# RuntimeRacer/vall-e

Measured on AMD Instinct MI355X. Metric: AR codec-tokens/sec/GPU + NAR 7-stage p50 latency, d=1024 L=12 10s utterance, higher is better.
Workload: dtype bf16

## Files before the change

### include/vallex.h

```cpp
#ifndef VALLEX_H
#define VALLEX_H

#include <stdint.h>

#ifdef __cplusplus
extern "C" {
#endif

typedef struct vx_engine vx_engine;

enum vx_status {
  VX_OK = 0,
  VX_ERR_ARG = 1,
  VX_ERR_HIP = 2,
  VX_ERR_STATE = 3,
  VX_ERR_CAPACITY = 4,
  VX_ERR_UNSUPPORTED = 5,
  VX_ERR_WEIGHTS = 6
};

enum vx_precision {
  VX_PREC_F32 = 0,
  VX_PREC_BF16 = 1,
  VX_PREC_FP8_NAR = 2
// ... 105 lines not shown

int vx_get_timings(vx_engine* e, double* out, int32_t n);

int vx_read_buffer(vx_engine* e, const char* name, void* dst, int64_t offset_bytes, int64_t nbytes);

int vx_buffer_bytes(const vx_config* cfg, const char* name, int64_t* bytes);

int vx_op_layernorm(int32_t prec, const float* x, const float* gamma, const float* beta, const float* ada_w,
                    const float* ada_b, void* out , int32_t rows, int32_t d, void* stream);
int vx_op_gemv(int32_t prec, const void* W, const float* bias, const float* x, float* y, int32_t N, int32_t K,
               int32_t relu, void* stream);
int vx_op_gemm(int32_t prec, int32_t use_mfma, const void* A, const void* W, const float* bias, float* C_f32,
               int32_t M, int32_t N, int32_t K, int32_t relu, void* stream);
int vx_op_gemm_rows(int32_t form, const void* A_bf16, const void* W_bf16, const float* bias, void* C, int32_t M, int32_t N,
                    int32_t K, int32_t relu, void* vt_bf16, int32_t vt_n0, int32_t vt_ld, void* stream);
int vx_op_gemm_mx(const float* A, const float* W, const float* bias, void* c_out, void* sc_out, int32_t M, int32_t N, int32_t K,
                  int32_t relu, int32_t out_mode, void* qa_out, void* sa_out, void* stream);
int vx_op_layernorm_mx(const float* x, const float* gamma, const float* beta, const float* ada_w, const float* ada_b, void* q_out,
                       void* s_out, int32_t rows, int32_t d, void* stream);
int vx_op_attention(int32_t prec, int32_t use_mfma, const void* qkv, void* out, int32_t rows, int32_t nhead,
                    int32_t hd, int32_t text_len_for_ar_mask , void* stream);
int vx_op_attention_segs(const void* qkv, void* out, int32_t rows, int32_t nhead, int32_t hd, int32_t nseg, const int32_t* seg_start,
                         const int32_t* seg_len, const int32_t* seg_text , void* stream);
int vx_op_cross_attention_segs(const void* q, int32_t ldq, const void* mem, const int64_t* mem_off, int64_t head_stride,
                               int64_t v_offset, const int32_t* klen, void* out, int32_t rows, int32_t nhead, int32_t nseg,
                               const int32_t* seg_start, const int32_t* seg_len, void* stream);
int vx_op_attn_slots(int32_t kv_fp8, const float* q, const void* kv, const void* kv_scale, int64_t slot_stride, int64_t v_offset,
                     int32_t ctx_max, int32_t B, int32_t nhead, const int32_t* ctx, const int32_t* done , void* out,
                     void* stream);
int vx_op_attn_mem_slots(const float* q, const void* mem, int64_t slot_stride, int64_t v_offset, int32_t max_text, int32_t B,
// ... 75 lines not shown
```

### vall-e_amd/csrc/engine.hip

```cpp
#include <hip/hip_runtime.h>

#include <cmath>
#include <cstdarg>
#include <cstdio>
#include <array>
#include <cstring>
#include <string>
#include <type_traits>
#include <unordered_map>
#include <vector>

#include "../../include/vallex.h"
#ifdef VX_STAMPS
__device__ unsigned long long g_vx_stamps[32];
__device__ unsigned long long* g_vx_kstamps = nullptr;
__device__ unsigned long long* g_fq_stamps = nullptr;
#endif
#include "ar_kernels.hpp"
#include "ar_tp.hpp"
#include "rows_kernels.hpp"
#include "mfma_kernels.hpp"
#include "batch_kernels.hpp"
#include "mx_kernels.hpp"

// ... 2006 lines not shown
    for (int i = 0; i < Q - 1; ++i) {
      for (int b = 0; b < n; ++b) {
        float* xb = e->X + (size_t)start[b] * dn;
        float* xa = xb + (size_t)tx[b] * dn;
        const float* ye = e->yemb + (size_t)aoff[b] * dn;
        const int A = P[b] + T[b];
        if (prenet) {
          if (!vf) HIPC(hipMemcpyAsync(xb, e->pn_text, (size_t)S2[b] * dn * 4, hipMemcpyDeviceToDevice, e->es));
          if (pos_before_prenet) {
            add_pos_kernel<<<A, 256, 0, e->es>>>(ye, dn, a_aud, e->pe_nar, 0, e->pn_a, A);
            VXC(audio_prenet_rows(e, 1, e->pn_a, xa, A, dn));
          } else {
            VXC(audio_prenet_rows(e, 1, ye, e->pn_b, A, dn));
            add_pos_kernel<<<A, 256, 0, e->es>>>(e->pn_b, dn, a_aud, e->pe_nar, 0, xa, A);
          }
        } else {
          if (!vf) embed_pos_kernel<<<S2[b], 256, 0, e->es>>>(e->ids_text + soff[b], 1, 0, W<float>(e, "nar_text_embedding.word_embeddings.weight"),
                                                              512, dn, a_txt, e->pe_nar, 0, xb, S2[b]);
          add_pos_kernel<<<A, 256, 0, e->es>>>(ye, dn, a_aud, e->pe_nar, 0, xa, A);
        }
      }
      VXC(run_stack(e, e->nar_l, rows, dn, c.nar_nhead, -1, i, segs, KvDst(), tmem));
      const float* fw = post ? nullptr : ada_vec(e, i, e->npl * c.nar_num_layers);
      for (int b = 0; b < n; ++b) {
        const float* xr = e->X + (size_t)(start[b] + tx[b] + P[b]) * dn;
        void* hr = (char*)e->Hn + (size_t)toff[b] * dn * e->esz;
        if (post) VXC(cast_rows(e, xr, hr, (size_t)T[b] * dn));
        else VXC(ln_rows(e, xr, W<float>(e, "nar_decoder.norm.norm.weight"), W<float>(e, "nar_decoder.norm.norm.bias"), fw, fw + dn, hr,
                         T[b], dn));
      }
      VXC(gemm_rows(e, e->Hn, W<void>(e, "nar_predict_layers." + std::to_string(i) + ".weight"), nullptr, e->nar_logits,
                    trows, 1024, dn, GE_PLAIN, true));
      argmax_rows_kernel<<<(trows + 3) / 4, 256, 0, e->es>>>(e->nar_logits, 1024, trows, e->ids_samples, e->d_codes, Q, i + 1);
      if (score) {
        nll_rows_kernel<<<(trows + NLL_ROWS_PER_WG - 1) / NLL_ROWS_PER_WG, 256, 0, e->es>>>(e->nar_logits, trows, 1024, 1024, e->d_fcodes, Q, i + 1,
                                                                                   e->sc_nll, e->sc_rank, nullptr);
        for (int b = 0; b < n; ++b) {
          if (score->nll) HIPC(hipMemcpyAsync(score->nll[b] + (size_t)i * T[b], e->sc_nll + toff[b], (size_t)T[b] * 4, hipMemcpyDefault, e->es));
          if (score->rank) HIPC(hipMemcpyAsync(score->rank[b] + (size_t)i * T[b], e->sc_rank + toff[b], (size_t)T[b] * 4, hipMemcpyDefault, e->es));
        }
      }
      if (stage_logits) HIPC(hipMemcpyAsync(stage_logits + (size_t)i * trows * 1024, e->nar_logits, (size_t)trows * 1024 * 4, hipMemcpyDefault, e->es));
      if (forced && i < Q - 2)
        pick_col_kernel<<<(trows + 255) / 256, 256, 0, e->es>>>(e->d_fcodes, Q, i + 1, e->ids_samples, trows);
      if (i < Q - 2)
        for (int b = 0; b < n; ++b) {
          float* ye = e->yemb + (size_t)aoff[b] * dn;
          if (c.prefix_mode == 0 && P[b])
            embed_accum_kernel<<<P[b], 256, 0, e->es>>>(e->ids_prompts + (size_t)aoff[b] * Q, Q, i + 1, emb(i + 1), 1024, dn, ye, P[b], 0);
          embed_accum_kernel<<<T[b], 256, 0, e->es>>>(e->ids_samples + toff[b], 1, 0, emb(i + 1), 1024, dn, ye + (size_t)P[b] * dn, T[b], 0);
        }
    }
  }
  HIPC(hipGetLastError());
  HIPC(hipEventRecord(e->ev_t[5], e->es));
  for (int b = 0; codes_out && b < n; ++b)
    HIPC(hipMemcpyAsync(codes_out[b], e->d_codes + (size_t)toff[b] * Q, (size_t)T[b] * Q * 8, hipMemcpyDefault, e->es));
  HIPC(hipStreamSynchronize(e->es));
  float ms = 0.f;
  HIPC(hipEventElapsedTime(&ms, e->ev_t[4], e->ev_t[5]));
  e->t_nar = ms;
  gemm_collect(e);
  e->last_T = trows; e->last_N = rows;
  VXC(sync_out(e, stream));
  return VX_OK;
// ... 418 lines not shown

extern "C" int vx_op_gemm_rows(int32_t form, const void* A, const void* Wp, const float* bias, void* C, int32_t M, int32_t N,
                               int32_t K, int32_t relu, void* vt, int32_t vt_n0, int32_t vt_ld, void* stream) {
  if (!A || !Wp || !C || !bias || M < 1 || N < 1 || K < 1) return fail(VX_ERR_ARG, "gemm_rows: null operand or empty shape");
  if (form != 0 && form != 1) return fail(VX_ERR_ARG, "gemm_rows: form %d", form);
  if (vt && (form != 0 || vt_n0 < 0 || vt_n0 >= N || vt_n0 % 64 != 0 || vt_ld < M))
    return fail(VX_ERR_ARG, "gemm_rows: V^T copy needs form 0, 0 <= vt_n0 < N, vt_n0 %% 64 == 0 (the kernels test whole column groups), vt_ld >= M");
  hipStream_t s = (hipStream_t)stream;
  if (mfma_gemm_dispatch((const bf16*)A, (const bf16*)Wp, bias, C, M, N, K, form == 1 ? GE_RESID : (relu ? GE_RELU : GE_BIAS), form == 1, s,
                         (bf16*)vt, vt_n0, vt_ld))
    return fail(VX_ERR_UNSUPPORTED, "gemm_rows: no kernel instance");
  HIPC(hipGetLastError());
  return VX_OK;
}

extern "C" int vx_op_gemm_mx(const float* A, const float* Wt, const float* bias, void* c_out, void* sc_out, int32_t M, int32_t N,
                             int32_t K, int32_t relu, int32_t out_mode, void* qa_out, void* sa_out, void* stream) {
  if (!A || !Wt || !c_out || M < 1 || N % 256 || K % 128) return fail(VX_ERR_UNSUPPORTED, "mx gemm: M=%d N=%d K=%d (N %% 256, K %% 128)", M, N, K);
  if (out_mode == 2 && !sc_out) return fail(VX_ERR_ARG, "mx gemm: out_mode 2 needs sc_out");
  hipStream_t s = (hipStream_t)stream;
  const int ld = (M + 255) / 256 * 256;
  struct Scratch {
    uint8_t *qa = nullptr, *sa = nullptr, *qw = nullptr, *sw = nullptr;
    ~Scratch() { (void)hipFree(qa); (void)hipFree(sa); (void)hipFree(qw); (void)hipFree(sw); }
  } t;
  HIPC(hipMalloc((void**)&t.qa, (size_t)M * K)); HIPC(hipMalloc((void**)&t.sa, (size_t)(K / 32) * ld));
  HIPC(hipMalloc((void**)&t.qw, (size_t)N * K)); HIPC(hipMalloc((void**)&t.sw, (size_t)(K / 32) * N));
  HIPC(hipMemsetAsync(t.sa, 0, (size_t)(K / 32) * ld, s));
  mx_quant_rows_kernel<<<(M + 3) / 4, 256, 0, s>>>(A, t.qa, t.sa, M, K, ld);
  mx_quant_rows_kernel<<<(N + 3) / 4, 256, 0, s>>>(Wt, t.qw, t.sw, N, K, N);
// ... 406 lines not shown
```

### vall-e_amd/csrc/mfma_kernels.hpp

```cpp
#pragma once
#include <cstdlib>
#include <type_traits>
#include <unordered_map>

#include "common.hpp"
#include "rows_kernels.hpp"

namespace vx {

typedef __bf16 bf16x8_t __attribute__((ext_vector_type(8)));
typedef float f32x16_t __attribute__((ext_vector_type(16)));

template <int EPI, bool OUT_F32, int RING>
__global__ __launch_bounds__(256) void mfma_gemm_kernel(const bf16* __restrict__ A, const bf16* __restrict__ W,
                                                        const float* __restrict__ bias, void* __restrict__ Cv, int M,
                                                        int N, int K, bf16* __restrict__ vt, int vt_n0, int vt_ld, int ld) {
  const int bx = blockIdx.x, by = blockIdx.y, bz = blockIdx.z;
  A += (size_t)bz * K;
  W += (size_t)bz * K;
  if (OUT_F32) Cv = reinterpret_cast<float*>(Cv) + (size_t)bz * M * N;
  constexpr int BM = 128, BN = 128;
  extern __shared__ __attribute__((aligned(16))) unsigned char lds[];
  const int tid = threadIdx.x, lane = tid & 63, wave = tid >> 6;
  const int wm = wave >> 1, wn = wave & 1;
  const int r = lane & 31, h = lane >> 5;
  const int m0 = by * BM, n0 = bx * BN;

  f32x16_t acc[2][2];
// ... 15 lines not shown
  constexpr int KS = RK / 16;
  constexpr int OPB = BM * RB;
  constexpr int NI = OPB / 4096;
  constexpr int ND = 2 * NI;
  auto swz = [](int row) { return RB == 128 ? ((row >> 1) & 7) : ((0 - (row >> 2)) & 3); };
  const int nk = K / RK;
  const int row0 = tid / CPR;
  const int csrc = ((tid % CPR) ^ swz(row0)) * 8;
  const bf16 *sA[NI], *sW[NI];
#pragma unroll
  for (int i = 0; i < NI; ++i) {
    sA[i] = A + (size_t)min(m0 + row0 + (256 / CPR) * i, M - 1) * ld + csrc;
    sW[i] = W + (size_t)min(n0 + row0 + (256 / CPR) * i, N - 1) * ld + csrc;
  }
  const int dbase = (tid - lane) * 16;
  auto stage = [&](int st) {
    unsigned char* base = lds + (st & 3) * (2 * OPB);
    const int k0 = st * RK;
#pragma unroll
    for (int i = 0; i < NI; ++i)
      __builtin_amdgcn_global_load_lds((const __attribute__((address_space(1))) void*)(sA[i] + k0),
                                       (__attribute__((address_space(3))) void*)(base + dbase + 4096 * i), 16, 0, 0);
#pragma unroll
    for (int i = 0; i < NI; ++i)
      __builtin_amdgcn_global_load_lds((const __attribute__((address_space(1))) void*)(sW[i] + k0),
                                       (__attribute__((address_space(3))) void*)(base + OPB + dbase + 4096 * i), 16, 0, 0);
  };
  bf16x8_t fa0[KS][2], fb0[KS][2], fa1[KS][2], fb1[KS][2];
  auto lread = [&](int st, bf16x8_t (&fa)[KS][2], bf16x8_t (&fb)[KS][2]) {
    const unsigned char* ba = lds + (st & 3) * (2 * OPB);
    const unsigned char* bw = ba + OPB;
#pragma unroll
    for (int ks = 0; ks < KS; ++ks)
#pragma unroll
      for (int i = 0; i < 2; ++i) {
        const int row = wm * 64 + i * 32 + r;
        fa[ks][i] = *reinterpret_cast<const bf16x8_t*>(ba + row * RB + (((ks * 2 + h) ^ swz(row)) << 4));
        const int col = wn * 64 + i * 32 + r;
        fb[ks][i] = *reinterpret_cast<const bf16x8_t*>(bw + col * RB + (((ks * 2 + h) ^ swz(col)) << 4));
      }
  };
  auto mm = [&](const bf16x8_t (&fa)[KS][2], const bf16x8_t (&fb)[KS][2]) {
#pragma unroll
    for (int ks = 0; ks < KS; ++ks)
#pragma unroll
      for (int i = 0; i < 2; ++i)
#pragma unroll
        for (int j = 0; j < 2; ++j) acc[i][j] = __builtin_amdgcn_mfma_f32_32x32x16_bf16(fa[ks][i], fb[ks][j], acc[i][j], 0, 0, 0);
  };
  auto steady = [&](int st, bf16x8_t (&fa)[KS][2], bf16x8_t (&fb)[KS][2], bf16x8_t (&na)[KS][2], bf16x8_t (&nb)[KS][2]) {
    stage(st + 3);
    lread(st + 1, na, nb);
    mm(fa, fb);
#pragma unroll
    for (int i = 0; i < ND; ++i) {
      __builtin_amdgcn_sched_group_barrier(0x010, 1, 0);
      __builtin_amdgcn_sched_group_barrier(0x008, 1, 0);
    }
#pragma unroll
    for (int i = 0; i < 4 * KS - ND; ++i) {
      __builtin_amdgcn_sched_group_barrier(0x100, 4 * KS / (4 * KS - ND), 0);
      __builtin_amdgcn_sched_group_barrier(0x008, 1, 0);
    }
    if (ND == 8) asm volatile("s_waitcnt vmcnt(8)\n\ts_barrier" ::: "memory");
    else asm volatile("s_waitcnt vmcnt(4)\n\ts_barrier" ::: "memory");
  };
  auto tail = [&](int st, bf16x8_t (&fa)[KS][2], bf16x8_t (&fb)[KS][2], bf16x8_t (&na)[KS][2], bf16x8_t (&nb)[KS][2]) {
    const bool more = st + 3 < nk;
    if (more) stage(st + 3);
    if (st + 1 < nk) lread(st + 1, na, nb);
    mm(fa, fb);
    if (more && ND == 8) asm volatile("s_waitcnt vmcnt(8)\n\ts_barrier" ::: "memory");
    else if (more) asm volatile("s_waitcnt vmcnt(4)\n\ts_barrier" ::: "memory");
    else asm volatile("s_waitcnt vmcnt(0)\n\ts_barrier" ::: "memory");
  };
  VX_STAMP(0);
  const int pre = nk < 3 ? nk : 3;
  for (int st = 0; st < pre; ++st) stage(st);
  VX_STAMP(1);
  if (pre == 3 && ND == 8) asm volatile("s_waitcnt vmcnt(8)\n\ts_barrier" ::: "memory");
  else if (pre == 3) asm volatile("s_waitcnt vmcnt(4)\n\ts_barrier" ::: "memory");
  else asm volatile("s_waitcnt vmcnt(0)\n\ts_barrier" ::: "memory");
  lread(0, fa0, fb0);
  VX_STAMP(2);
  int st = 0;
  for (; st + 4 < nk; st += 2) {
    steady(st, fa0, fb0, fa1, fb1);
    steady(st + 1, fa1, fb1, fa0, fb0);
  }
  VX_STAMP(3);
  for (; st < nk; st += 2) {
    tail(st, fa0, fb0, fa1, fb1);
    if (st + 1 < nk) tail(st + 1, fa1, fb1, fa0, fb0);
  }
  VX_STAMP(4);
  asm volatile("" : "+v"(bias_r[0]), "+v"(bias_r[1]));

  if constexpr (!OUT_F32) {
    constexpr int LDT = 136;
    bf16* tile = reinterpret_cast<bf16*>(lds);
#pragma unroll
    for (int j = 0; j < 2; ++j) {
      const int nl = wn * 64 + j * 32 + r;
      const float bv = bias_r[j];
#pragma unroll
      for (int i = 0; i < 2; ++i)
#pragma unroll
        for (int v = 0; v < 16; ++v) {
          const int ml = wm * 64 + i * 32 + (v & 3) + 8 * (v >> 2) + 4 * h;
// ... 49 lines not shown
    for (int j = 0; j < 2; ++j) {
      const int n = n0 + wn * 64 + j * 32 + r;
      const float bv = bias_r[j];
#pragma unroll
      for (int i = 0; i < 2; ++i) {
#pragma unroll
        for (int v = 0; v < 16; ++v) {
          const int m = m0 + wm * 64 + i * 32 + (v & 3) + 8 * (v >> 2) + 4 * h;
          if (m < M && n < N) {
            float x = acc[i][j][v] + bv;
            if (EPI == GE_RELU) x = fmaxf(x, 0.f);
            float* c = reinterpret_cast<float*>(Cv) + (size_t)m * N + n;
            *c = (EPI == GE_RESID) ? (*c + x) : x;
          }
        }
      }
    }
  }
  VX_STAMP(5);
}

template <int EPI, bool OUT_F32, int SPLITK>
__global__ __launch_bounds__(256) void wgemm_kernel(const bf16* __restrict__ A, const bf16* __restrict__ W,
                                                    const float* __restrict__ bias, void* __restrict__ Cv, int M, int N,
                                                    int K, bf16* __restrict__ vt, int vt_n0, int vt_ld, int ngroups,
                                                    int ngroups_pad) {
  extern __shared__ __attribute__((aligned(16))) unsigned char lds[];
  const int tid = threadIdx.x, lane = tid & 63, wave = tid >> 6;
  const int r = lane & 31, h = lane >> 5;
  const int ng = blockIdx.x % ngroups_pad, mt = blockIdx.x / ngroups_pad;
// ... 625 lines not shown
  for (int c = 8; c >= 2; c >>= 1)
    if (rem * c <= grid && nk % (2 * c) == 0 && nk / c >= 8) { S = c; break; }
  if (S == 0) return tl;
  const float full = 1.5f * nk, split = 1.5f * nk / S + (float)rem * S * 0.262144f * 2.f / 4.f + 7.f;
  if (split > 0.7f * full) return tl;
  hipStreamCaptureStatus cs = hipStreamCaptureStatusNone;
  if (hipStreamIsCapturing(s, &cs) != hipSuccess || cs != hipStreamCaptureStatusNone) return tl;
  static std::unordered_map<hipStream_t, float*> wss;
  float*& w = wss[s];
  if (w == nullptr && hipMalloc((void**)&w, (size_t)256 * 262144) != hipSuccess) { w = nullptr; return tl; }
  tl.ws = w;
  tl.split = S;
  return tl;
}

static inline int mfma_gemm_dispatch(const bf16* A, const bf16* W, const float* bias, void* C, int M, int N, int K,
                                     int epi, bool out_f32, hipStream_t s, bf16* vt = nullptr, int vt_n0 = 0,
                                     int vt_ld = 0) {
  if (K % 64 != 0 || N % 64 != 0) {
    gemm_simple_launch(A, W, bias, C, M, N, K, epi, out_f32, s);
    return 0;
  }
  const long long tiles64 = (long long)((M + 63) / 64) * (N / 64);
  if (M >= 4096 && N % 256 == 0 && K >= 128) {
    const int ntn = N / 256, ntm = (M + 255) / 256, nt_all = ntn * ntm;
    const int ncu = vx_cu_count();
    const int grid256 = nt_all < ncu ? nt_all : ncu;
    const bool p8 = K % 128 == 0 && (size_t)M * K * 2 < 0xFFFF0000ull && (size_t)N * K * 2 < 0xFFFF0000ull;
    const P8Tail tl = p8 ? p8_tail_plan(nt_all, grid256, K, s) : P8Tail{nullptr, 0};
    gemm_epi_dispatch(epi, out_f32, [&](auto E, auto F) {
// ... 8 lines not shown
        attr_done = true;
      }
      if (p8 && tl.split > 1) {
        const int rem_t = nt_all % grid256;
        mfma256p_kernel<EPI, OUT_F32, true><<<grid256, 512, 131072 + 2048, s>>>(A, W, bias, C, M, N, K, vt, vt_n0, vt_ld, ntn, nt_all, tl);
        p8_tail_reduce_kernel<EPI, OUT_F32><<<dim3(rem_t, 16), 256, 0, s>>>(tl.ws, tl.split, nt_all - rem_t, ntn, nt_all, bias, C, M, N, vt, vt_n0, vt_ld);
      } else if (p8) {
        mfma256p_kernel<EPI, OUT_F32><<<grid256, 512, 131072 + 2048, s>>>(A, W, bias, C, M, N, K, vt, vt_n0, vt_ld, ntn, nt_all, tl);
      } else {
        mfma256_kernel<EPI, OUT_F32><<<grid256, 512, 131072, s>>>(A, W, bias, C, M, N, K, vt, vt_n0, vt_ld, ntn, nt_all);
      }
    });
    return 0;
  }
  if (N % 128 == 0 && tiles64 >= 512) {
    const dim3 grid(N / 128, (M + 127) / 128);
    const int ring = gemm_ring128((long long)grid.x * grid.y);
    gemm_epi_dispatch(epi, out_f32, [&](auto E, auto F) {
      constexpr int EPI = decltype(E)::value;
      constexpr bool OUT_F32 = decltype(F)::value;
      static bool attr_dev[16] = {};
      bool& attr_done = attr_dev[vx_cur_device()];
      if (!attr_done) {
        (void)hipFuncSetAttribute((const void*)mfma_gemm_kernel<EPI, OUT_F32, 64>, hipFuncAttributeMaxDynamicSharedMemorySize, 131072);
        (void)hipFuncSetAttribute((const void*)mfma_gemm_kernel<EPI, OUT_F32, 32>, hipFuncAttributeMaxDynamicSharedMemorySize, 65536);
        attr_done = true;
      }
      if (ring == 64) mfma_gemm_kernel<EPI, OUT_F32, 64><<<grid, 256, 131072, s>>>(A, W, bias, C, M, N, K, vt, vt_n0, vt_ld, K);
      else mfma_gemm_kernel<EPI, OUT_F32, 32><<<grid, 256, 65536, s>>>(A, W, bias, C, M, N, K, vt, vt_n0, vt_ld, K);
    });
    return 0;
  }
  const int mtiles = (M + 63) / 64;
  const size_t lds = 131072;
  const bool split = (K % 256 == 0) && tiles64 < 512;
  gemm_epi_dispatch(epi, out_f32, [&](auto E, auto F) {
    constexpr int EPI = decltype(E)::value;
    constexpr bool OUT_F32 = decltype(F)::value;
    auto launch = [&](auto SPLITK) {
      constexpr int S = decltype(SPLITK)::value;
      static bool attr_dev[16] = {};
      bool& attr_done = attr_dev[vx_cur_device()];
      if (!attr_done) {
        (void)hipFuncSetAttribute((const void*)wgemm_kernel<EPI, OUT_F32, S>, hipFuncAttributeMaxDynamicSharedMemorySize, (int)lds);
        attr_done = true;
      }
      const int ngr = (S == 1) ? (N + 255) / 256 : N / 64;
      const int ngp = (ngr + 7) / 8 * 8;
      wgemm_kernel<EPI, OUT_F32, S><<<mtiles * ngp, 256, lds, s>>>(A, W, bias, C, M, N, K, vt, vt_n0, vt_ld, ngr, ngp);
    };
    if (split) launch(std::integral_constant<int, 4>{});
    else launch(std::integral_constant<int, 1>{});
  });
  return 0;
}

static inline int mfma_gemm_partial(const bf16* A, const bf16* W, float* slabs, int M, int N, int K, int splits, hipStream_t s) {
  static bool attr_dev[16] = {}; bool& attr_done = attr_dev[vx_cur_device()];
  if (!attr_done) {
    (void)hipFuncSetAttribute((const void*)mfma_gemm_kernel<GE_PLAIN, true, 64>, hipFuncAttributeMaxDynamicSharedMemorySize, 131072);
    (void)hipFuncSetAttribute((const void*)mfma_gemm_kernel<GE_PLAIN, true, 32>, hipFuncAttributeMaxDynamicSharedMemorySize, 65536);
    attr_done = true;
  }
  dim3 grid(N / 128, (M + 127) / 128, splits);
  if (gemm_ring128((long long)grid.x * grid.y * grid.z) == 64)
    mfma_gemm_kernel<GE_PLAIN, true, 64><<<grid, 256, 131072, s>>>(A, W, nullptr, slabs, M, N, K / splits, nullptr, 0, 0, K);
  else
    mfma_gemm_kernel<GE_PLAIN, true, 32><<<grid, 256, 65536, s>>>(A, W, nullptr, slabs, M, N, K / splits, nullptr, 0, 0, K);
  return 0;
}

__device__ __forceinline__ float xor32_f(float v) {
  const auto r = __builtin_amdgcn_permlane32_swap(__builtin_bit_cast(unsigned, v), __builtin_bit_cast(unsigned, v), false, false);
  return __builtin_bit_cast(float, (threadIdx.x & 32) ? r[0] : r[1]);
}

template <int NW, int KG>
__global__ __launch_bounds__(NW * KG * 64, (KG == 2 ? 2 : 1)) void mfma_attn_kernel(const bf16* __restrict__ qkv, const bf16* __restrict__ vt,
                                                                 bf16* __restrict__ out, int M, int vt_ld, int d,
                                                                 int text_len, const int* __restrict__ seg_start,
// ... 478 lines not shown
```

### vall-e_amd/csrc/rows_kernels.hpp

```cpp
#pragma once
#include <type_traits>

#include "common.hpp"

namespace vx {

__global__ __launch_bounds__(256) void embed_pos_kernel(const long long* __restrict__ ids, int id_stride, int id_off,
                                                        const float* __restrict__ table, int table_rows, int d,
                                                        const float* __restrict__ alpha, const float* __restrict__ pe,
                                                        int pos0, float* __restrict__ out, int rows) {
  const int r = blockIdx.x;
  if (r >= rows) return;
  const long long id = min(max(ids[(size_t)r * id_stride + id_off], 0ll), (long long)table_rows - 1);
  const float al = alpha[0];
  for (int c = threadIdx.x; c < d; c += 256)
    out[(size_t)r * d + c] = __fadd_rn(table[(size_t)id * d + c], __fmul_rn(al, pe[(size_t)(pos0 + r) * d + c]));
}

__global__ __launch_bounds__(256) void add_pos_kernel(const float* __restrict__ src, int d,
                                                      const float* __restrict__ alpha, const float* __restrict__ pe,
                                                      int pos0, float* __restrict__ out, int rows) {
  const int r = blockIdx.x;
  if (r >= rows) return;
  const float al = alpha[0];
  for (int c = threadIdx.x; c < d; c += 256)
    out[(size_t)r * d + c] = __fadd_rn(src[(size_t)r * d + c], __fmul_rn(al, pe[(size_t)(pos0 + r) * d + c]));
}

__global__ __launch_bounds__(256) void embed_accum_kernel(const long long* __restrict__ ids, int id_stride, int id_off,
                                                          const float* __restrict__ table, int table_rows, int d,
                                                          float* __restrict__ acc, int rows, int init) {
  const int r = blockIdx.x;
  if (r >= rows) return;
  const long long id = min(max(ids[(size_t)r * id_stride + id_off], 0ll), (long long)table_rows - 1);
  for (int c = threadIdx.x; c < d; c += 256) {
    const float e = table[(size_t)id * d + c];
    acc[(size_t)r * d + c] = init ? e : __fadd_rn(acc[(size_t)r * d + c], e);
  }
}

constexpr int CONV_TT = 4;
// ... 386 lines not shown
  const int j = blockIdx.x, z = blockIdx.y;
  if (j >= seg_len[z]) return;
  const size_t r = (size_t)seg_start[z] + j;
  T* kc = kv_layer + (size_t)seg_slot[z] * slot_stride;
  T* vc = kc + v_offset;
  for (int i = threadIdx.x; i < d; i += 256) {
    const int h = i / hd, c = i - h * hd;
    const size_t dst = ((size_t)h * ctx_max + j) * hd + c;
    kc[dst] = qkv[r * 3 * d + d + i];
    vc[dst] = qkv[r * 3 * d + 2 * d + i];
  }
}

__global__ __launch_bounds__(256) void argmax_rows_kernel(const float* __restrict__ logits, int N, int rows,
                                                          long long* __restrict__ samples,
                                                          long long* __restrict__ codes, int Q, int col) {
  const int lane = threadIdx.x & 63;
  const int r = blockIdx.x * 4 + (threadIdx.x >> 6);
  if (r >= rows) return;
  ValIdx best{-INFINITY, 0x7fffffff};
  for (int i = lane; i < N; i += 64) {
    ValIdx c{logits[(size_t)r * N + i], i};
    best = better(best, c);
  }
  best = wave_argmax(best);
  if (lane == 0) {
    samples[r] = best.i;
    codes[(size_t)r * Q + col] = best.i;
  }
}

constexpr int NLL_MAXV = 1088, NLL_ROWS_PER_WG = 4;
__global__ __launch_bounds__(256) void nll_rows_kernel(const float* __restrict__ logits, int rows, int V, int ld,
                                                       const long long* __restrict__ targets, int t_stride, int t_off,
                                                       float* __restrict__ nll, int* __restrict__ rank, int* __restrict__ argmax) {
  constexpr int NV = NLL_MAXV / 64;
  const int lane = threadIdx.x & 63;
  const int r = blockIdx.x * NLL_ROWS_PER_WG + (threadIdx.x >> 6);
  if (r >= rows) return;
  const float* row = logits + (size_t)r * ld;
  const long long t_raw = targets[(size_t)r * t_stride + t_off];
  const bool t_ok = t_raw >= 0 && t_raw < V;
  const int t = t_ok ? (int)t_raw : 0;
// ... 68 lines not shown
```

### vall-e_amd/engine.py

```python
from __future__ import annotations

import ctypes as C
import os
from typing import Optional

import numpy as np
import torch

_HERE = os.path.dirname(os.path.abspath(__file__))
LIB_PATH = os.path.join(_HERE, "csrc", "libvallex.so")

VX_PREC_F32, VX_PREC_BF16, VX_PREC_FP8_NAR = 0, 1, 2
BMAX = 64
VX_FLAG_TRACE_LOGITS, VX_FLAG_NO_GRAPH, VX_FLAG_SIMPLE_ROWS, VX_FLAG_POST_NORM, VX_FLAG_PRENET, VX_FLAG_VALLF = 1, 2, 4, 8, 16, 32
VX_FLAG_KV_FP8 = 64
VX_FLAG_VALLF_ROWS = 128
KV_CACHES = ("bf16", "fp8")
VX_ADMIT_BATCHED, VX_ADMIT_PER_SLOT = 0, 1
VX_CODEC_LSTM_GRAPH, VX_CODEC_ENCODER = 1, 2
BE_QKV, BE_RELU, BE_PARTIAL, BE_LOGITS, BE_LOGITS_MAP, BE_BIAS = range(6)
STOP_REASONS = {0: "none", 1: "eos_argmax", 2: "eos_sample", 3: "length", 4: "max_new"}


class VxConfig(C.Structure):
# ... 47 lines not shown
    "vx_batch_admit": (C.c_int, [C.c_void_p, C.c_int32, C.POINTER(C.c_int32), C.POINTER(C.c_void_p), C.POINTER(C.c_int32),
                                 C.POINTER(C.c_void_p), C.POINTER(C.c_int32), C.POINTER(VxDecodeParams), C.c_int32, C.c_void_p]),
    "vx_batch_run": (C.c_int, [C.c_void_p, C.c_int32, C.c_int32, C.POINTER(C.c_int32), C.POINTER(C.c_int32), C.c_void_p]),
    "vx_nar_batch": (C.c_int, [C.c_void_p, C.c_int32] + [C.c_void_p] * 7 + [C.c_void_p]),
    "vx_nar_batch_ex": (C.c_int, [C.c_void_p, C.c_int32] + [C.c_void_p] * 8 + [C.c_void_p]),
    "vx_score": (C.c_int, [C.c_void_p, C.c_void_p, C.c_int32, C.c_void_p, C.c_int32, C.c_void_p, C.c_int32, C.c_int32]
                 + [C.c_void_p] * 4 + [C.c_void_p]),
    "vx_score_batch": (C.c_int, [C.c_void_p, C.c_int32] + [C.c_void_p] * 11 + [C.c_void_p]),
    "vx_get_timings": (C.c_int, [C.c_void_p, C.POINTER(C.c_double), C.c_int32]),
    "vx_read_buffer": (C.c_int, [C.c_void_p, C.c_char_p, C.c_void_p, C.c_int64, C.c_int64]),
    "vx_buffer_bytes": (C.c_int, [C.c_void_p, C.c_char_p, C.POINTER(C.c_int64)]),
    "vx_op_layernorm": (C.c_int, [C.c_int32] + [C.c_void_p] * 6 + [C.c_int32, C.c_int32, C.c_void_p]),
    "vx_op_gemv": (C.c_int, [C.c_int32] + [C.c_void_p] * 4 + [C.c_int32, C.c_int32, C.c_int32, C.c_void_p]),
    "vx_op_gemm": (C.c_int, [C.c_int32, C.c_int32] + [C.c_void_p] * 4 + [C.c_int32] * 4 + [C.c_void_p]),
    "vx_op_gemm_rows": (C.c_int, [C.c_int32] + [C.c_void_p] * 4 + [C.c_int32] * 4 + [C.c_void_p, C.c_int32, C.c_int32, C.c_void_p]),
    "vx_op_gemm_mx": (C.c_int, [C.c_void_p] * 5 + [C.c_int32] * 5 + [C.c_void_p] * 3),
    "vx_op_layernorm_mx": (C.c_int, [C.c_void_p] * 7 + [C.c_int32, C.c_int32, C.c_void_p]),
    "vx_op_attention": (C.c_int, [C.c_int32, C.c_int32, C.c_void_p, C.c_void_p] + [C.c_int32] * 4 + [C.c_void_p]),
    "vx_op_attention_segs": (C.c_int, [C.c_void_p, C.c_void_p] + [C.c_int32] * 4 + [C.POINTER(C.c_int32)] * 3 + [C.c_void_p]),
    "vx_op_cross_attention_segs": (C.c_int, [C.c_void_p, C.c_int32, C.c_void_p, C.POINTER(C.c_int64), C.c_int64, C.c_int64,
                                             C.POINTER(C.c_int32), C.c_void_p] + [C.c_int32] * 3 + [C.POINTER(C.c_int32)] * 2 + [C.c_void_p]),
    "vx_op_attn_slots": (C.c_int, [C.c_int32] + [C.c_void_p] * 3 + [C.c_int64, C.c_int64] + [C.c_int32] * 3
                         + [C.POINTER(C.c_int32)] * 2 + [C.c_void_p, C.c_void_p]),
    "vx_op_attn_mem_slots": (C.c_int, [C.c_void_p, C.c_void_p, C.c_int64, C.c_int64] + [C.c_int32] * 3
                             + [C.POINTER(C.c_int32)] * 2 + [C.c_void_p, C.c_void_p]),
    "vx_op_bgemm": (C.c_int, [C.c_int32, C.c_int32] + [C.c_void_p] * 3 + [C.c_int32] * 4 + [C.POINTER(C.c_int32)] * 3
                    + [C.c_void_p] * 3 + [C.c_int64, C.c_int64, C.c_int32, C.c_int32] + [C.c_void_p] * 3 + [C.c_int32, C.c_void_p,
                    C.c_int32, C.POINTER(C.c_int32), C.c_void_p]),
    "vx_op_ln_batch": (C.c_int, [C.c_void_p, C.c_void_p, C.c_int32] + [C.c_void_p] * 4 + [C.c_int32, C.c_int32, C.POINTER(C.c_int32),
                       C.c_void_p]),
# ... 401 lines not shown
def op_gemm_rows(A, W, bias, relu=False, resid=None, vt_cols=0):
    lib = load_library()
    M, K = A.shape
    N = W.shape[0]
    if resid is not None:
        _check(lib.vx_op_gemm_rows(1, _ptr(A), _ptr(W), _ptr(bias), _ptr(resid), M, N, K, 0, None, 0, 0, current_stream_ptr(A.device)))
        return resid
    Cm = torch.empty((M, N), dtype=torch.bfloat16, device=A.device)
    ld = (M + 255) // 256 * 256
    vt = torch.zeros((vt_cols, ld), dtype=torch.bfloat16, device=A.device) if vt_cols else None
    _check(lib.vx_op_gemm_rows(0, _ptr(A), _ptr(W), _ptr(bias), _ptr(Cm), M, N, K, int(relu), _ptr(vt), N - vt_cols, ld,
                               current_stream_ptr(A.device)))
    return Cm, vt


def op_gemm_mx(A, W, bias=None, relu=False, out_mx=False, return_quant=False):
    lib = load_library()
    M, K = A.shape
    N = W.shape[0]
    ld = (M + 255) // 256 * 256
    dev = A.device
    if out_mx:
        c = torch.empty((M, N), dtype=torch.uint8, device=dev)
        sc = torch.empty((N // 32, ld), dtype=torch.uint8, device=dev)
    else:
        c, sc = torch.empty((M, N), dtype=torch.float32, device=dev), None
    qa = torch.empty((M, K), dtype=torch.uint8, device=dev) if return_quant else None
    sa = torch.empty((K // 32, ld), dtype=torch.uint8, device=dev) if return_quant else None
    _check(lib.vx_op_gemm_mx(_ptr(A), _ptr(W), _ptr(bias), _ptr(c), _ptr(sc), M, N, K, int(relu), 2 if out_mx else 0, _ptr(qa), _ptr(sa),
                             current_stream_ptr(dev)))
# ... 160 lines not shown
```

Before: 4592.

## Fold ragged M remainder into last tile row of 128 GEMM; fuse NAR embed steps

Adds a STRIP variant of the 128x128 MFMA GEMM. When M leaves a small remainder (1-16 rows) that would push the grid just past the CU count, the last block row also computes the remainder rows with an extra MFMA per k-step, staged through an additional LDS ring. This avoids a second, mostly idle wave of workgroups. It also fuses NAR text-embedding and audio-position kernels into one launch, and folds the next-stage embedding accumulation into argmax for single-utterance runs. The cost is extra LDS, register pressure and scheduling complexity in the strip kernel.

```diff
diff --git a/include/vallex.h b/include/vallex.h
--- a/include/vallex.h
+++ b/include/vallex.h
@@ -143,6 +143,8 @@
                int32_t M, int32_t N, int32_t K, int32_t relu, void* stream);
 int vx_op_gemm_rows(int32_t form, const void* A_bf16, const void* W_bf16, const float* bias, void* C, int32_t M, int32_t N,
                     int32_t K, int32_t relu, void* vt_bf16, int32_t vt_n0, int32_t vt_ld, void* stream);
+int vx_op_gemm_tile128(int32_t form, const void* A_bf16, const void* W_bf16, const float* bias, void* C, int32_t M, int32_t N, int32_t K,
+                       int32_t relu, void* vt_bf16, int32_t vt_n0, int32_t vt_ld, int32_t splits, int32_t strip, void* stream);
 int vx_op_gemm_mx(const float* A, const float* W, const float* bias, void* c_out, void* sc_out, int32_t M, int32_t N, int32_t K,
                   int32_t relu, int32_t out_mode, void* qa_out, void* sa_out, void* stream);
 int vx_op_layernorm_mx(const float* x, const float* gamma, const float* beta, const float* ada_w, const float* ada_b, void* q_out,
diff --git a/vall-e_amd/csrc/engine.hip b/vall-e_amd/csrc/engine.hip
--- a/vall-e_amd/csrc/engine.hip
+++ b/vall-e_amd/csrc/engine.hip
@@ -2044,9 +2044,10 @@
             VXC(audio_prenet_rows(e, 1, ye, e->pn_b, A, dn));
             add_pos_kernel<<<A, 256, 0, e->es>>>(e->pn_b, dn, a_aud, e->pe_nar, 0, xa, A);
           }
+        } else if (!vf) {
+          nar_stage_rows_kernel<<<S2[b] + A, 256, 0, e->es>>>(e->ids_text + soff[b], W<float>(e, "nar_text_embedding.word_embeddings.weight"), 512,
+                                                              dn, a_txt, a_aud, e->pe_nar, ye, xb, S2[b], A);
         } else {
-          if (!vf) embed_pos_kernel<<<S2[b], 256, 0, e->es>>>(e->ids_text + soff[b], 1, 0, W<float>(e, "nar_text_embedding.word_embeddings.weight"),
-                                                              512, dn, a_txt, e->pe_nar, 0, xb, S2[b]);
           add_pos_kernel<<<A, 256, 0, e->es>>>(ye, dn, a_aud, e->pe_nar, 0, xa, A);
         }
       }
@@ -2061,7 +2062,12 @@
       }
       VXC(gemm_rows(e, e->Hn, W<void>(e, "nar_predict_layers." + std::to_string(i) + ".weight"), nullptr, e->nar_logits,
                     trows, 1024, dn, GE_PLAIN, true));
-      argmax_rows_kernel<<<(trows + 3) / 4, 256, 0, e->es>>>(e->nar_logits, 1024, trows, e->ids_samples, e->d_codes, Q, i + 1);
+      const bool fuse_emb = n == 1 && !forced && i < Q - 2;
+      if (fuse_emb)
+        argmax_rows_kernel<<<(trows + 3) / 4, 256, 0, e->es>>>(e->nar_logits, 1024, trows, e->ids_samples, e->d_codes, Q, i + 1, emb(i + 1), 1024,
+                                                               dn, e->yemb + (size_t)P[0] * dn);
+      else
+        argmax_rows_kernel<<<(trows + 3) / 4, 256, 0, e->es>>>(e->nar_logits, 1024, trows, e->ids_samples, e->d_codes, Q, i + 1);
       if (score) {
         nll_rows_kernel<<<(trows + NLL_ROWS_PER_WG - 1) / NLL_ROWS_PER_WG, 256, 0, e->es>>>(e->nar_logits, trows, 1024, 1024, e->d_fcodes, Q, i + 1,
                                                                                    e->sc_nll, e->sc_rank, nullptr);
@@ -2078,7 +2084,8 @@
           float* ye = e->yemb + (size_t)aoff[b] * dn;
           if (c.prefix_mode == 0 && P[b])
             embed_accum_kernel<<<P[b], 256, 0, e->es>>>(e->ids_prompts + (size_t)aoff[b] * Q, Q, i + 1, emb(i + 1), 1024, dn, ye, P[b], 0);
-          embed_accum_kernel<<<T[b], 256, 0, e->es>>>(e->ids_samples + toff[b], 1, 0, emb(i + 1), 1024, dn, ye + (size_t)P[b] * dn, T[b], 0);
+          if (!fuse_emb)
+            embed_accum_kernel<<<T[b], 256, 0, e->es>>>(e->ids_samples + toff[b], 1, 0, emb(i + 1), 1024, dn, ye + (size_t)P[b] * dn, T[b], 0);
         }
     }
   }
@@ -2527,6 +2534,25 @@
   return VX_OK;
 }
 
+extern "C" int vx_op_gemm_tile128(int32_t form, const void* A, const void* Wp, const float* bias, void* C, int32_t M, int32_t N,
+                                  int32_t K, int32_t relu, void* vt, int32_t vt_n0, int32_t vt_ld, int32_t splits, int32_t strip,
+                                  void* stream) {
+  if (!A || !Wp || !C || M < 1 || N < 1 || K < 1) return fail(VX_ERR_ARG, "gemm_tile128: null operand or empty shape");
+  if (form < 0 || form > 2 || (form != 2 && !bias)) return fail(VX_ERR_ARG, "gemm_tile128: form %d", form);
+  if (form != 2) splits = 1;
+  if (splits != 1 && splits != 2 && splits != 4) return fail(VX_ERR_ARG, "gemm_tile128: splits %d", splits);
+  if (N % 128 != 0 || K % (64 * splits) != 0) return fail(VX_ERR_UNSUPPORTED, "gemm_tile128: N %d, K %d, splits %d", N, K, splits);
+  if (strip && (M < 128 || M % 128 < 1 || M % 128 > 16)) return fail(VX_ERR_ARG, "gemm_tile128: no strip at M = %d", M);
+  if (vt && (form != 0 || vt_n0 < 0 || vt_n0 >= N || vt_n0 % 128 != 0 || vt_ld < (M + 127) / 128 * 128))
+    return fail(VX_ERR_ARG, "gemm_tile128: V^T copy needs form 0, vt_n0 a multiple of 128 below N, vt_ld >= M rounded up to 128");
+  hipStream_t s = (hipStream_t)stream;
+  if (form == 2) mfma_gemm_partial((const bf16*)A, (const bf16*)Wp, (float*)C, M, N, K, splits, s, strip ? 1 : 0);
+  else mfma_gemm128_launch((const bf16*)A, (const bf16*)Wp, bias, C, M, N, K, form == 1 ? GE_RESID : (relu ? GE_RELU : GE_BIAS), form == 1,
+                           strip != 0, s, (bf16*)vt, vt_n0, vt_ld);
+  HIPC(hipGetLastError());
+  return VX_OK;
+}
+
 extern "C" int vx_op_gemm_mx(const float* A, const float* Wt, const float* bias, void* c_out, void* sc_out, int32_t M, int32_t N,
                              int32_t K, int32_t relu, int32_t out_mode, void* qa_out, void* sa_out, void* stream) {
   if (!A || !Wt || !c_out || M < 1 || N % 256 || K % 128) return fail(VX_ERR_UNSUPPORTED, "mx gemm: M=%d N=%d K=%d (N %% 256, K %% 128)", M, N, K);
diff --git a/vall-e_amd/csrc/mfma_kernels.hpp b/vall-e_amd/csrc/mfma_kernels.hpp
--- a/vall-e_amd/csrc/mfma_kernels.hpp
+++ b/vall-e_amd/csrc/mfma_kernels.hpp
@@ -11,7 +11,7 @@
 typedef __bf16 bf16x8_t __attribute__((ext_vector_type(8)));
 typedef float f32x16_t __attribute__((ext_vector_type(16)));
 
-template <int EPI, bool OUT_F32, int RING>
+template <int EPI, bool OUT_F32, int RING, bool STRIP = false>
 __global__ __launch_bounds__(256) void mfma_gemm_kernel(const bf16* __restrict__ A, const bf16* __restrict__ W,
                                                         const float* __restrict__ bias, void* __restrict__ Cv, int M,
                                                         int N, int K, bf16* __restrict__ vt, int vt_n0, int vt_ld, int ld) {
@@ -57,85 +57,110 @@
     sW[i] = W + (size_t)min(n0 + row0 + (256 / CPR) * i, N - 1) * ld + csrc;
   }
   const int dbase = (tid - lane) * 16;
-  auto stage = [&](int st) {
-    unsigned char* base = lds + (st & 3) * (2 * OPB);
-    const int k0 = st * RK;
-#pragma unroll
-    for (int i = 0; i < NI; ++i)
-      __builtin_amdgcn_global_load_lds((const __attribute__((address_space(1))) void*)(sA[i] + k0),
-                                       (__attribute__((address_space(3))) void*)(base + dbase + 4096 * i), 16, 0, 0);
-#pragma unroll
-    for (int i = 0; i < NI; ++i)
-      __builtin_amdgcn_global_load_lds((const __attribute__((address_space(1))) void*)(sW[i] + k0),
-                                       (__attribute__((address_space(3))) void*)(base + OPB + dbase + 4096 * i), 16, 0, 0);
-  };
-  bf16x8_t fa0[KS][2], fb0[KS][2], fa1[KS][2], fb1[KS][2];
-  auto lread = [&](int st, bf16x8_t (&fa)[KS][2], bf16x8_t (&fb)[KS][2]) {
-    const unsigned char* ba = lds + (st & 3) * (2 * OPB);
-    const unsigned char* bw = ba + OPB;
-#pragma unroll
-    for (int ks = 0; ks < KS; ++ks)
-#pragma unroll
-      for (int i = 0; i < 2; ++i) {
-        const int row = wm * 64 + i * 32 + r;
-        fa[ks][i] = *reinterpret_cast<const bf16x8_t*>(ba + row * RB + (((ks * 2 + h) ^ swz(row)) << 4));
-        const int col = wn * 64 + i * 32 + r;
-        fb[ks][i] = *reinterpret_cast<const bf16x8_t*>(bw + col * RB + (((ks * 2 + h) ^ swz(col)) << 4));
-      }
-  };
-  auto mm = [&](const bf16x8_t (&fa)[KS][2], const bf16x8_t (&fb)[KS][2]) {
-#pragma unroll
-    for (int ks = 0; ks < KS; ++ks)
-#pragma unroll
-      for (int i = 0; i < 2; ++i)
-#pragma unroll
-        for (int j = 0; j < 2; ++j) acc[i][j] = __builtin_amdgcn_mfma_f32_32x32x16_bf16(fa[ks][i], fb[ks][j], acc[i][j], 0, 0, 0);
-  };
-  auto steady = [&](int st, bf16x8_t (&fa)[KS][2], bf16x8_t (&fb)[KS][2], bf16x8_t (&na)[KS][2], bf16x8_t (&nb)[KS][2]) {
-    stage(st + 3);
-    lread(st + 1, na, nb);
-    mm(fa, fb);
-#pragma unroll
-    for (int i = 0; i < ND; ++i) {
-      __builtin_amdgcn_sched_group_barrier(0x010, 1, 0);
-      __builtin_amdgcn_sched_group_barrier(0x008, 1, 0);
-    }
-#pragma unroll
-    for (int i = 0; i < 4 * KS - ND; ++i) {
-      __builtin_amdgcn_sched_group_barrier(0x100, 4 * KS / (4 * KS - ND), 0);
-      __builtin_amdgcn_sched_group_barrier(0x008, 1, 0);
-    }
-    if (ND == 8) asm volatile("s_waitcnt vmcnt(8)\n\ts_barrier" ::: "memory");
-    else asm volatile("s_waitcnt vmcnt(4)\n\ts_barrier" ::: "memory");
-  };
-  auto tail = [&](int st, bf16x8_t (&fa)[KS][2], bf16x8_t (&fb)[KS][2], bf16x8_t (&na)[KS][2], bf16x8_t (&nb)[KS][2]) {
-    const bool more = st + 3 < nk;
-    if (more) stage(st + 3);
-    if (st + 1 < nk) lread(st + 1, na, nb);
-    mm(fa, fb);
-    if (more && ND == 8) asm volatile("s_waitcnt vmcnt(8)\n\ts_barrier" ::: "memory");
-    else if (more) asm volatile("s_waitcnt vmcnt(4)\n\ts_barrier" ::: "memory");
-    else asm volatile("s_waitcnt vmcnt(0)\n\ts_barrier" ::: "memory");
-  };
+  static_assert(!STRIP || RING == 64, "the strip is staged as 32 rows of 128 bytes: one LDS-DMA instruction of the workgroup");
+  const bool strip = STRIP && by == (int)gridDim.y - 1;
+  const int ms0 = (M / BM) * BM;
+  const bf16* sS = A + (size_t)min(ms0 + row0, M - 1) * ld + csrc;
+  unsigned char* const lds_strip = lds + 4 * (2 * OPB);
+  const int wm_u = __builtin_amdgcn_readfirstlane(wm);
+  f32x16_t accs;
+#pragma unroll
+  for (int v = 0; v < 16; ++v) accs[v] = 0.f;
   VX_STAMP(0);
-  const int pre = nk < 3 ? nk : 3;
-  for (int st = 0; st < pre; ++st) stage(st);
-  VX_STAMP(1);
-  if (pre == 3 && ND == 8) asm volatile("s_waitcnt vmcnt(8)\n\ts_barrier" ::: "memory");
-  else if (pre == 3) asm volatile("s_waitcnt vmcnt(4)\n\ts_barrier" ::: "memory");
-  else asm volatile("s_waitcnt vmcnt(0)\n\ts_barrier" ::: "memory");
-  lread(0, fa0, fb0);
-  VX_STAMP(2);
-  int st = 0;
-  for (; st + 4 < nk; st += 2) {
-    steady(st, fa0, fb0, fa1, fb1);
-    steady(st + 1, fa1, fb1, fa0, fb0);
-  }
-  VX_STAMP(3);
-  for (; st < nk; st += 2) {
-    tail(st, fa0, fb0, fa1, fb1);
-    if (st + 1 < nk) tail(st + 1, fa1, fb1, fa0, fb0);
-  }
+  auto kloop = [&](auto strip_c) {
+    constexpr bool S = decltype(strip_c)::value;
+    constexpr int NDS = ND + (S ? 1 : 0);
+    constexpr int NMM = (S ? 5 : 4) * KS;
+    struct Frag { bf16x8_t a[KS][2], b[KS][2], s[KS]; };
+    auto stage = [&](int st) {
+      unsigned char* base = lds + (st & 3) * (2 * OPB);
+      const int k0 = st * RK;
+#pragma unroll
+      for (int i = 0; i < NI; ++i)
+        __builtin_amdgcn_global_load_lds((const __attribute__((address_space(1))) void*)(sA[i] + k0),
+                                         (__attribute__((address_space(3))) void*)(base + dbase + 4096 * i), 16, 0, 0);
+#pragma unroll
+      for (int i = 0; i < NI; ++i)
+        __builtin_amdgcn_global_load_lds((const __attribute__((address_space(1))) void*)(sW[i] + k0),
+                                         (__attribute__((address_space(3))) void*)(base + OPB + dbase + 4096 * i), 16, 0, 0);
+      if (S)
+        __builtin_amdgcn_global_load_lds((const __attribute__((address_space(1))) void*)(sS + k0),
+                                         (__attribute__((address_space(3))) void*)(lds_strip + (st & 3) * 4096 + dbase), 16, 0, 0);
+    };
+    auto lread = [&](int st, Frag& f) {
+      const unsigned char* ba = lds + (st & 3) * (2 * OPB);
+      const unsigned char* bw = ba + OPB;
+#pragma unroll
+      for (int ks = 0; ks < KS; ++ks) {
+#pragma unroll
+        for (int i = 0; i < 2; ++i) {
+          const int row = wm * 64 + i * 32 + r;
+          f.a[ks][i] = *reinterpret_cast<const bf16x8_t*>(ba + row * RB + (((ks * 2 + h) ^ swz(row)) << 4));
+          const int col = wn * 64 + i * 32 + r;
+          f.b[ks][i] = *reinterpret_cast<const bf16x8_t*>(bw + col * RB + (((ks * 2 + h) ^ swz(col)) << 4));
+        }
+        if (S) f.s[ks] = *reinterpret_cast<const bf16x8_t*>(lds_strip + (st & 3) * 4096 + r * RB + (((ks * 2 + h) ^ swz(r)) << 4));
+      }
+    };
+    auto mm = [&](const Frag& f) {
+#pragma unroll
+      for (int ks = 0; ks < KS; ++ks) {
+#pragma unroll
+        for (int i = 0; i < 2; ++i)
+#pragma unroll
+          for (int j = 0; j < 2; ++j) acc[i][j] = __builtin_amdgcn_mfma_f32_32x32x16_bf16(f.a[ks][i], f.b[ks][j], acc[i][j], 0, 0, 0);
+        if (S) accs = __builtin_amdgcn_mfma_f32_32x32x16_bf16(f.s[ks], wm_u ? f.b[ks][1] : f.b[ks][0], accs, 0, 0, 0);
+      }
+    };
+    auto wait_bar = [&](bool more) {
+      if (!more) asm volatile("s_waitcnt vmcnt(0)\n\ts_barrier" ::: "memory");
+      else if (NDS == 9) asm volatile("s_waitcnt vmcnt(9)\n\ts_barrier" ::: "memory");
+      else if (NDS == 8) asm volatile("s_waitcnt vmcnt(8)\n\ts_barrier" ::: "memory");
+      else asm volatile("s_waitcnt vmcnt(4)\n\ts_barrier" ::: "memory");
+    };
+    auto steady = [&](int st, const Frag& f, Frag& nf) {
+      stage(st + 3);
+      lread(st + 1, nf);
+      mm(f);
+#pragma unroll
+      for (int i = 0; i < NDS; ++i) {
+        __builtin_amdgcn_sched_group_barrier(0x010, 1, 0);
+        __builtin_amdgcn_sched_group_barrier(0x008, 1, 0);
+      }
+#pragma unroll
+      for (int i = 0; i < NMM - NDS; ++i) {
+        __builtin_amdgcn_sched_group_barrier(0x100, (NMM + NMM - NDS - 1) / (NMM - NDS), 0);
+        __builtin_amdgcn_sched_group_barrier(0x008, 1, 0);
+      }
+      wait_bar(true);
+    };
+    auto tail = [&](int st, const Frag& f, Frag& nf) {
+      const bool more = st + 3 < nk;
+      if (more) stage(st + 3);
+      if (st + 1 < nk) lread(st + 1, nf);
+      mm(f);
+      wait_bar(more);
+    };
+    Frag f0, f1;
+    const int pre = nk < 3 ? nk : 3;
+    for (int st = 0; st < pre; ++st) stage(st);
+    VX_STAMP(1);
+    wait_bar(pre == 3);
+    lread(0, f0);
+    VX_STAMP(2);
+    int st = 0;
+    for (; st + 4 < nk; st += 2) {
+      steady(st, f0, f1);
+      steady(st + 1, f1, f0);
+    }
+    VX_STAMP(3);
+    for (; st < nk; st += 2) {
+      tail(st, f0, f1);
+      if (st + 1 < nk) tail(st + 1, f1, f0);
+    }
+  };
+  if (strip) kloop(std::true_type{});
+  else kloop(std::false_type{});
   VX_STAMP(4);
   asm volatile("" : "+v"(bias_r[0]), "+v"(bias_r[1]));
 
@@ -215,6 +240,26 @@
             *c = (EPI == GE_RESID) ? (*c + x) : x;
           }
         }
+      }
+    }
+  }
+  if (strip) {
+    const int n = n0 + wn * 64 + wm * 32 + r;
+    const float bv = wm_u ? bias_r[1] : bias_r[0];
+    const bool to_vt = !OUT_F32 && vt != nullptr && n0 >= vt_n0;
+#pragma unroll
+    for (int v = 0; v < 8; ++v) {
+      const int m = ms0 + (v & 3) + 8 * (v >> 2) + 4 * h;
+      float x = accs[v] + bv;
+      if (EPI == GE_RELU) x = fmaxf(x, 0.f);
+      if constexpr (OUT_F32) {
+        if (m < M) {
+          float* c = reinterpret_cast<float*>(Cv) + (size_t)m * N + n;
+          *c = (EPI == GE_RESID) ? (*c + x) : x;
+        }
+      } else {
+        if (m < M) reinterpret_cast<bf16*>(Cv)[(size_t)m * N + n] = (bf16)x;
+        if (to_vt && m < vt_ld) vt[(size_t)(n - vt_n0) * vt_ld + m] = (bf16)x;
       }
     }
   }
@@ -870,6 +915,33 @@
   return tl;
 }
 
+static inline bool gemm_strip128(int M, long long per_row) {
+  const int rem = M % 128;
+  if (M < 128 || rem < 1 || rem > 16) return false;
+  return per_row * ((M + 127) / 128) > vx_cu_count() && per_row * (M / 128) <= vx_cu_count();
+}
+
+static inline void mfma_gemm128_launch(const bf16* A, const bf16* W, const float* bias, void* C, int M, int N, int K, int epi,
+                                       bool out_f32, bool strip, hipStream_t s, bf16* vt, int vt_n0, int vt_ld) {
+  const dim3 grid(N / 128, strip ? M / 128 : (M + 127) / 128);
+  const int ring = strip ? 64 : gemm_ring128((long long)grid.x * grid.y);
+  gemm_epi_dispatch(epi, out_f32, [&](auto E, auto F) {
+    constexpr int EPI = decltype(E)::value;
+    constexpr bool OUT_F32 = decltype(F)::value;
+    static bool attr_dev[16] = {};
+    bool& attr_done = attr_dev[vx_cur_device()];
+    if (!attr_done) {
+      (void)hipFuncSetAttribute((const void*)mfma_gemm_kernel<EPI, OUT_F32, 64>, hipFuncAttributeMaxDynamicSharedMemorySize, 131072);
+      (void)hipFuncSetAttribute((const void*)mfma_gemm_kernel<EPI, OUT_F32, 32>, hipFuncAttributeMaxDynamicSharedMemorySize, 65536);
+      (void)hipFuncSetAttribute((const void*)mfma_gemm_kernel<EPI, OUT_F32, 64, true>, hipFuncAttributeMaxDynamicSharedMemorySize, 131072 + 16384);
+      attr_done = true;
+    }
+    if (strip) mfma_gemm_kernel<EPI, OUT_F32, 64, true><<<grid, 256, 131072 + 16384, s>>>(A, W, bias, C, M, N, K, vt, vt_n0, vt_ld, K);
+    else if (ring == 64) mfma_gemm_kernel<EPI, OUT_F32, 64><<<grid, 256, 131072, s>>>(A, W, bias, C, M, N, K, vt, vt_n0, vt_ld, K);
+    else mfma_gemm_kernel<EPI, OUT_F32, 32><<<grid, 256, 65536, s>>>(A, W, bias, C, M, N, K, vt, vt_n0, vt_ld, K);
+  });
+}
+
 static inline int mfma_gemm_dispatch(const bf16* A, const bf16* W, const float* bias, void* C, int M, int N, int K,
                                      int epi, bool out_f32, hipStream_t s, bf16* vt = nullptr, int vt_n0 = 0,
                                      int vt_ld = 0) {
@@ -908,21 +980,7 @@
     return 0;
   }
   if (N % 128 == 0 && tiles64 >= 512) {
-    const dim3 grid(N / 128, (M + 127) / 128);
-    const int ring = gemm_ring128((long long)grid.x * grid.y);
-    gemm_epi_dispatch(epi, out_f32, [&](auto E, auto F) {
-      constexpr int EPI = decltype(E)::value;
-      constexpr bool OUT_F32 = decltype(F)::value;
-      static bool attr_dev[16] = {};
-      bool& attr_done = attr_dev[vx_cur_device()];
-      if (!attr_done) {
-        (void)hipFuncSetAttribute((const void*)mfma_gemm_kernel<EPI, OUT_F32, 64>, hipFuncAttributeMaxDynamicSharedMemorySize, 131072);
-        (void)hipFuncSetAttribute((const void*)mfma_gemm_kernel<EPI, OUT_F32, 32>, hipFuncAttributeMaxDynamicSharedMemorySize, 65536);
-        attr_done = true;
-      }
-      if (ring == 64) mfma_gemm_kernel<EPI, OUT_F32, 64><<<grid, 256, 131072, s>>>(A, W, bias, C, M, N, K, vt, vt_n0, vt_ld, K);
-      else mfma_gemm_kernel<EPI, OUT_F32, 32><<<grid, 256, 65536, s>>>(A, W, bias, C, M, N, K, vt, vt_n0, vt_ld, K);
-    });
+    mfma_gemm128_launch(A, W, bias, C, M, N, K, epi, out_f32, gemm_strip128(M, N / 128), s, vt, vt_n0, vt_ld);
     return 0;
   }
   const int mtiles = (M + 63) / 64;
@@ -949,15 +1007,21 @@
   return 0;
 }
 
-static inline int mfma_gemm_partial(const bf16* A, const bf16* W, float* slabs, int M, int N, int K, int splits, hipStream_t s) {
+static inline int mfma_gemm_partial(const bf16* A, const bf16* W, float* slabs, int M, int N, int K, int splits, hipStream_t s,
+                                    int strip = -1) {
   static bool attr_dev[16] = {}; bool& attr_done = attr_dev[vx_cur_device()];
   if (!attr_done) {
     (void)hipFuncSetAttribute((const void*)mfma_gemm_kernel<GE_PLAIN, true, 64>, hipFuncAttributeMaxDynamicSharedMemorySize, 131072);
     (void)hipFuncSetAttribute((const void*)mfma_gemm_kernel<GE_PLAIN, true, 32>, hipFuncAttributeMaxDynamicSharedMemorySize, 65536);
+    (void)hipFuncSetAttribute((const void*)mfma_gemm_kernel<GE_PLAIN, true, 64, true>, hipFuncAttributeMaxDynamicSharedMemorySize, 131072 + 16384);
     attr_done = true;
   }
-  dim3 grid(N / 128, (M + 127) / 128, splits);
-  if (gemm_ring128((long long)grid.x * grid.y * grid.z) == 64)
+  const bool st = strip < 0 ? gemm_strip128(M, (long long)(N / 128) * splits) : strip != 0;
+  dim3 grid(N / 128, st ? M / 128 : (M + 127) / 128, splits);
+  const int ring = st ? 64 : gemm_ring128((long long)grid.x * grid.y * grid.z);
+  if (st)
+    mfma_gemm_kernel<GE_PLAIN, true, 64, true><<<grid, 256, 131072 + 16384, s>>>(A, W, nullptr, slabs, M, N, K / splits, nullptr, 0, 0, K);
+  else if (ring == 64)
     mfma_gemm_kernel<GE_PLAIN, true, 64><<<grid, 256, 131072, s>>>(A, W, nullptr, slabs, M, N, K / splits, nullptr, 0, 0, K);
   else
     mfma_gemm_kernel<GE_PLAIN, true, 32><<<grid, 256, 65536, s>>>(A, W, nullptr, slabs, M, N, K / splits, nullptr, 0, 0, K);
diff --git a/vall-e_amd/csrc/rows_kernels.hpp b/vall-e_amd/csrc/rows_kernels.hpp
--- a/vall-e_amd/csrc/rows_kernels.hpp
+++ b/vall-e_amd/csrc/rows_kernels.hpp
@@ -25,6 +25,25 @@
   const float al = alpha[0];
   for (int c = threadIdx.x; c < d; c += 256)
     out[(size_t)r * d + c] = __fadd_rn(src[(size_t)r * d + c], __fmul_rn(al, pe[(size_t)(pos0 + r) * d + c]));
+}
+
+__global__ __launch_bounds__(256) void nar_stage_rows_kernel(const long long* __restrict__ ids, const float* __restrict__ table,
+                                                             int table_rows, int d, const float* __restrict__ a_txt,
+                                                             const float* __restrict__ a_aud, const float* __restrict__ pe,
+                                                             const float* __restrict__ yemb, float* __restrict__ out, int S, int A) {
+  const int r = blockIdx.x;
+  if (r >= S + A) return;
+  if (r < S) {
+    const long long id = min(max(ids[r], 0ll), (long long)table_rows - 1);
+    const float al = a_txt[0];
+    for (int c = threadIdx.x; c < d; c += 256)
+      out[(size_t)r * d + c] = __fadd_rn(table[(size_t)id * d + c], __fmul_rn(al, pe[(size_t)r * d + c]));
+  } else {
+    const int ra = r - S;
+    const float al = a_aud[0];
+    for (int c = threadIdx.x; c < d; c += 256)
+      out[(size_t)r * d + c] = __fadd_rn(yemb[(size_t)ra * d + c], __fmul_rn(al, pe[(size_t)ra * d + c]));
+  }
 }
 
 __global__ __launch_bounds__(256) void embed_accum_kernel(const long long* __restrict__ ids, int id_stride, int id_off,
@@ -441,7 +460,9 @@
 
 __global__ __launch_bounds__(256) void argmax_rows_kernel(const float* __restrict__ logits, int N, int rows,
                                                           long long* __restrict__ samples,
-                                                          long long* __restrict__ codes, int Q, int col) {
+                                                          long long* __restrict__ codes, int Q, int col,
+                                                          const float* __restrict__ table = nullptr, int table_rows = 0, int d = 0,
+                                                          float* __restrict__ acc = nullptr) {
   const int lane = threadIdx.x & 63;
   const int r = blockIdx.x * 4 + (threadIdx.x >> 6);
   if (r >= rows) return;
@@ -454,6 +475,10 @@
   if (lane == 0) {
     samples[r] = best.i;
     codes[(size_t)r * Q + col] = best.i;
+  }
+  if (table != nullptr) {
+    const int id = min(max(best.i, 0), table_rows - 1);
+    for (int c = lane; c < d; c += 64) acc[(size_t)r * d + c] = __fadd_rn(acc[(size_t)r * d + c], table[(size_t)id * d + c]);
   }
 }
 
diff --git a/vall-e_amd/engine.py b/vall-e_amd/engine.py
--- a/vall-e_amd/engine.py
+++ b/vall-e_amd/engine.py
@@ -85,6 +85,7 @@
     "vx_op_gemv": (C.c_int, [C.c_int32] + [C.c_void_p] * 4 + [C.c_int32, C.c_int32, C.c_int32, C.c_void_p]),
     "vx_op_gemm": (C.c_int, [C.c_int32, C.c_int32] + [C.c_void_p] * 4 + [C.c_int32] * 4 + [C.c_void_p]),
     "vx_op_gemm_rows": (C.c_int, [C.c_int32] + [C.c_void_p] * 4 + [C.c_int32] * 4 + [C.c_void_p, C.c_int32, C.c_int32, C.c_void_p]),
+    "vx_op_gemm_tile128": (C.c_int, [C.c_int32] + [C.c_void_p] * 4 + [C.c_int32] * 4 + [C.c_void_p] + [C.c_int32] * 4 + [C.c_void_p]),
     "vx_op_gemm_mx": (C.c_int, [C.c_void_p] * 5 + [C.c_int32] * 5 + [C.c_void_p] * 3),
     "vx_op_layernorm_mx": (C.c_int, [C.c_void_p] * 7 + [C.c_int32, C.c_int32, C.c_void_p]),
     "vx_op_attention": (C.c_int, [C.c_int32, C.c_int32, C.c_void_p, C.c_void_p] + [C.c_int32] * 4 + [C.c_void_p]),
@@ -516,6 +517,25 @@
     return Cm, vt
 
 
+def op_gemm_tile128(A, W, bias, strip, relu=False, resid=None, splits=0, vt_cols=0, out=None):
+    lib = load_library()
+    M, K = A.shape
+    N = W.shape[0]
+    st = current_stream_ptr(A.device)
+    if splits:
+        Cm = out if out is not None else torch.empty((splits, M, N), dtype=torch.float32, device=A.device)
+        _check(lib.vx_op_gemm_tile128(2, _ptr(A), _ptr(W), None, _ptr(Cm), M, N, K, 0, None, 0, 0, splits, int(strip), st))
+        return Cm
+    if resid is not None:
+        _check(lib.vx_op_gemm_tile128(1, _ptr(A), _ptr(W), _ptr(bias), _ptr(resid), M, N, K, 0, None, 0, 0, 1, int(strip), st))
+        return resid
+    Cm = out if out is not None else torch.empty((M, N), dtype=torch.bfloat16, device=A.device)
+    ld = (M + 255) // 256 * 256
+    vt = torch.zeros((vt_cols, ld), dtype=torch.bfloat16, device=A.device) if vt_cols else None
+    _check(lib.vx_op_gemm_tile128(0, _ptr(A), _ptr(W), _ptr(bias), _ptr(Cm), M, N, K, int(relu), _ptr(vt), N - vt_cols, ld, 1, int(strip), st))
+    return Cm, vt
+
+
 def op_gemm_mx(A, W, bias=None, relu=False, out_mx=False, return_quant=False):
     lib = load_library()
     M, K = A.shape
```

Measured after the change: 4565. Within noise of the previous version (-0.6%).
